# tachitachi/SR-WaveNet

Measured on NVIDIA B200. Metric: audio samples/sec, higher is better.
Workload: dtype f16

## Files before the change

sr-wavenet_b200/csrc/fused_bf16.cu:

```cuda
#include "common.cuh"
#include "mol.cuh"
#include "umma.cuh"
#include "philox.cuh"
#include <cuda_fp16.h>
#include <algorithm>
#include <cstdlib>

const float* srwn_host_weights(srwn_ctx* c);
__global__ void k_cond(const float* __restrict__ enc, const float* __restrict__ cond_k,
                       const float* __restrict__ cond_b, float* __restrict__ cond,
                       int frames_total, int L, int C);

namespace fused {

constexpr int kTile = 128;
#ifndef SRWN_STUDENT_TILES
#define SRWN_STUDENT_TILES 4
#endif
__host__ __device__ constexpr int tiles_of(bool teacher) { return teacher ? 3 : SRWN_STUDENT_TILES; }
__host__ __device__ constexpr int chunk_of(bool teacher) { return kTile * tiles_of(teacher); }
constexpr int kHalo = 512;
constexpr int kMaxLayers = 40;
constexpr int kMaxSeg = 8;

constexpr int kWfBytes = 64 * 32 * 2;
constexpr int kWrsTeacher = 32 * 160 * 2;
constexpr int kWrsStudent = 32 * 32 * 2;
constexpr int kH1Bytes = 128 * 128 * 2;
constexpr int kH2Bytes = 128 * 32 * 2;

struct Seg { int b, t_start, t_out, t_end; };

struct Params {
  const uint8_t* packed;
  const float* x_in;
  const float* x_scored;
  const float* cb;
  uint8_t* rings;
  const Seg* segs;
  const int* nseg;
  uint32_t* flags;
  int G;
  long long wait_limit;
  NoiseSpec noise;
  float* logits_out;
  float* nll_out;
  double* nll_partial;
  float* scale_out;
  float* mean_out;
  float* x_out;
  int* err;
#ifdef SRWN_TUNING
  long long* trace;
  int trace_chunk;
#endif
  int T, L, P, frames, O, M;
  int ring_bytes_per_team;
  int dil[kMaxLayers];
  int ring_off[kMaxLayers];
  int rsuf[kMaxLayers + 1];
};

template <bool TEACHER>
struct SmemMapT {
  static constexpr int NT = tiles_of(TEACHER);
  static constexpr int rows = kHalo + NT * kTile;
  static constexpr int hbuf = 0;
  static constexpr int hbuf_bytes = 4 * rows * 16;
  static constexpr int cbuf = hbuf + 2 * hbuf_bytes;
  static constexpr int cbuf_bytes = 4 * kTile * 16;
  static constexpr int wst = cbuf + NT * cbuf_bytes;
  static constexpr int wst_bytes = kWfBytes + (TEACHER ? kWrsTeacher : kWrsStudent);
  static constexpr int head = wst + 2 * wst_bytes;
  static constexpr int bias = head + (TEACHER ? kH1Bytes + kH2Bytes : 0);
  static constexpr int hbias = bias + kMaxLayers * 32 * 4;
  static constexpr int front = hbias + (128 + 128 + 32 + 64 + 4) * 4;
  static constexpr int cbs = front + 64 * 4;
  static constexpr int bars = cbs + NT * (kMaxLayers + 1) * 32 * 4;
  static constexpr int n_bars = 40;
  static constexpr int misc = bars + n_bars * 8;
  static constexpr int total = misc + 64;
};
static_assert(SmemMapT<true>::total <= 232448 && SmemMapT<false>::total <= 232448, "shared memory budget");
static_assert(3 * 16 * kTile * 16 <= 2 * SmemMapT<true>::hbuf_bytes, "head operand overlay");

template <int NT>
struct BarT {
  static constexpr int D1 = 0;
  static constexpr int D2 = NT;
  static constexpr int HD = 2 * NT;
  static constexpr int WFULL = 4 * NT;
  static constexpr int WEMPTY = WFULL + 2;
  static constexpr int HALO = WFULL + 4;
  static constexpr int G1 = WFULL + 6;
  static constexpr int HDD = WFULL + 8;
  static constexpr int TAIL = HDD + NT;
  static constexpr int C2 = TAIL + 1;
  static constexpr int count = C2 + 2 * NT;
};
static_assert(BarT<3>::count <= 40 && BarT<4>::count <= 40, "barrier slots");

using namespace umma;

template <bool FP16>
__device__ __forceinline__ uint32_t gate2(f2_t a) {
  float a0, a1;
  upk(a, a0, a1);
#if SRWN_EXP & 2
  return pack2<FP16>(a0, a1);
#endif
  const f2_t f = pk(tanh_fast(a0), tanh_fast(a1));
  const f2_t s = mul2(f, f);
  f2_t t = fma2(s, pk(0.0017294071149080992f, 0.0017294071149080992f), pk(-0.020638039335608482f, -0.020638039335608482f));
  t = fma2(s, t, pk(0.2499687224626541f, 0.2499687224626541f));
  const f2_t c = fma2(f, pk(0.5f, 0.5f), mul2(s, t));
  float c0, c1;
  upk(c, c0, c1);
  return pack2<FP16>(c0, c1);
}

template <bool FP16>
__device__ __forceinline__ void store_row(uint8_t* buf, int rows_per_kc, int row, const float* v) {
#pragma unroll
  for (int kc = 0; kc < 4; kc++) {
    uint4 q;
    q.x = pack2<FP16>(v[kc * 8 + 0], v[kc * 8 + 1]); q.y = pack2<FP16>(v[kc * 8 + 2], v[kc * 8 + 3]);
    q.z = pack2<FP16>(v[kc * 8 + 4], v[kc * 8 + 5]); q.w = pack2<FP16>(v[kc * 8 + 6], v[kc * 8 + 7]);
    *reinterpret_cast<uint4*>(buf + ((size_t)kc * rows_per_kc + row) * 16) = q;
  }
}
__device__ __forceinline__ void store_row_packed(uint8_t* buf, int rows_per_kc, int row, const uint32_t* w) {
#pragma unroll
  for (int kc = 0; kc < 4; kc++)
    *reinterpret_cast<uint4*>(buf + ((size_t)kc * rows_per_kc + row) * 16) =
        make_uint4(w[kc * 4 + 0], w[kc * 4 + 1], w[kc * 4 + 2], w[kc * 4 + 3]);
}

#ifndef SRWN_EXP
#define SRWN_EXP 0
#endif
#if !defined(SRWN_TUNING) || !(SRWN_EXP & 16)
#define TRACE(role, layer, slot) do {} while (0)
#else
#define TRACE(role, layer, slot)                                                            \
  do {                                                                                      \
    if (tracing) p.trace[((role) * kMaxLayers + (layer)) * 12 + (slot)] = clock64();      \
  } while (0)
#endif

#if SRWN_EXP & 1
#define LOOP_FENCE() do {} while (0)
#else
#define LOOP_FENCE() fence_async_smem()
#endif

constexpr int kLoadWarp = 0;
__host__ __device__ constexpr int threads_of(bool handoff, int nt) { return (1 + 4 * nt + (handoff ? 1 : 0)) * 32; }

__device__ __noinline__ bool flag_spin(const uint32_t* f, uint32_t need, volatile int* abort_flag, const int* gerr, int code, long long limit) {
  const long long t0 = clock64();
  int spins = 0;
  uint32_t v;
  while (true) {
    __nanosleep(32);
    asm volatile("ld.acquire.gpu.global.u32 %0, [%1];" : "=r"(v) : "l"(f) : "memory");
    if (v >= need) return true;
    if (*abort_flag) return false;
    if (((++spins) & 1023) == 0 && *reinterpret_cast<const volatile int*>(gerr)) return false;
    if (clock64() - t0 > limit) {
      if (atomicCAS((int*)abort_flag, 0, 1) == 0) ((int*)abort_flag)[1] = code;
      return false;
    }
  }
}
__device__ __forceinline__ bool flag_try(const uint32_t* f, uint32_t need) {
  uint32_t v;
  asm volatile("ld.acquire.gpu.global.u32 %0, [%1];" : "=r"(v) : "l"(f) : "memory");
  if (v < need) return false;
  asm volatile("fence.proxy.async;" ::: "memory");
  return true;
}
__device__ __forceinline__ bool flag_wait(const uint32_t* f, uint32_t need, volatile int* abort_flag, const int* gerr, int code, long long limit) {
  uint32_t v;
  asm volatile("ld.acquire.gpu.global.u32 %0, [%1];" : "=r"(v) : "l"(f) : "memory");
  if (v < need && !flag_spin(f, need, abort_flag, gerr, code, limit)) return false;
  asm volatile("fence.proxy.async;" ::: "memory");
  return true;
}
__device__ __forceinline__ void ring_rows_done(uint32_t counter_addr, uint32_t rows) {
  asm volatile("red.release.cta.shared::cta.add.u32 [%0], %1;" ::"r"(counter_addr), "r"(rows) : "memory");
}
__device__ __forceinline__ int ring_rows_of(int d, int m, int chunk) {
  const int lo = max(chunk - d, m * kTile), hi = (m + 1) * kTile;
  return hi > lo ? hi - lo : 0;
}
__device__ __forceinline__ uint32_t ld_acquire_cta_shared(uint32_t addr) {
  uint32_t v;
  asm volatile("ld.acquire.cta.shared::cta.u32 %0, [%1];" : "=r"(v) : "r"(addr) : "memory");
  return v;
}
__device__ __forceinline__ void flag_publish(uint32_t* f, uint32_t chunks) {
  asm volatile("red.release.gpu.global.max.u32 [%0], %1;" ::"l"(f), "r"(chunks) : "memory");
}

template <bool TEACHER, bool FP16, bool HANDOFF>
__global__ void __launch_bounds__(threads_of(HANDOFF, tiles_of(TEACHER)), 1) k_fused(const Params p) {
  constexpr int NT = tiles_of(TEACHER), CH = NT * kTile;
  constexpr int kThreads = threads_of(HANDOFF, NT);
  constexpr int kPubWarp = 1 + 4 * NT;
  constexpr int TCOLS = TEACHER ? 160 : 64;
  using SM = SmemMapT<TEACHER>;
  constexpr int ROWS = SM::rows;
  using BR = BarT<NT>;
  constexpr int BAR_D1 = BR::D1, BAR_D2 = BR::D2, BAR_HD = BR::HD, BAR_WFULL = BR::WFULL, BAR_WEMPTY = BR::WEMPTY, BAR_HALO = BR::HALO,
                BAR_G1 = BR::G1, BAR_HDD = BR::HDD, BAR_TAIL = BR::TAIL, BAR_C2 = BR::C2;
  (void)BAR_HDD; (void)BAR_C2; (void)kPubWarp;
  extern __shared__ __align__(1024) uint8_t smem[];
  const int tid = threadIdx.x, lane = tid & 31, warp = tid >> 5;
  const uint32_t sbase = smem_u32(smem);
  volatile int* abort_flag = reinterpret_cast<volatile int*>(smem + SM::misc + 8);
  uint32_t* tmem_slot = reinterpret_cast<uint32_t*>(smem + SM::misc);
  auto bar = [&](int i) { return sbase + SM::bars + i * 8; };
  const int L = p.L;
  constexpr int wrs_bytes = TEACHER ? kWrsTeacher : kWrsStudent;
  constexpr int layer_bytes = kWfBytes + wrs_bytes;
  constexpr int wrs_rows = TEACHER ? 160 : 32;

  if (tid == 0) {
    for (int i = 0; i < NT; i++) {
      mbar_init(bar(BAR_D1 + i), 1); mbar_init(bar(BAR_D2 + i), 1); mbar_init(bar(BAR_HDD + i), 1);
      mbar_init(bar(BAR_C2 + 2 * i), 1); mbar_init(bar(BAR_C2 + 2 * i + 1), 1);
      mbar_init(bar(BAR_HD + 2 * i), kTile); mbar_init(bar(BAR_HD + 2 * i + 1), kTile);
    }
    for (int i = 0; i < 2; i++) {
      mbar_init(bar(BAR_WFULL + i), 1); mbar_init(bar(BAR_WEMPTY + i), NT);
      mbar_init(bar(BAR_HALO + i), 1); mbar_init(bar(BAR_G1 + i), NT);
    }
    mbar_init(bar(BAR_TAIL), 1);
    abort_flag[0] = 0; abort_flag[1] = 0;
    for (int i = 0; i < NT; i++) reinterpret_cast<volatile uint32_t*>(smem + SM::misc + 16)[i] = 0;
    asm volatile("fence.mbarrier_init.release.cluster;" ::: "memory");
  }
  {
    const uint8_t* pk_ = p.packed;
    const size_t off_fixed = (size_t)L * layer_bytes;
    const float* fbias = reinterpret_cast<const float*>(pk_ + off_fixed);
    float* s_bias = reinterpret_cast<float*>(smem + SM::bias);
    for (int i = tid; i < L * 32; i += kThreads) s_bias[i] = fbias[i];
    const float* ffront = fbias + kMaxLayers * 32;
    float* s_front = reinterpret_cast<float*>(smem + SM::front);
    for (int i = tid; i < 64; i += kThreads) s_front[i] = ffront[i];
    const float* fhb = ffront + 64;
    float* s_hb = reinterpret_cast<float*>(smem + SM::hbias);
    for (int i = tid; i < 128 + 128 + 32 + 64 + 4; i += kThreads) s_hb[i] = fhb[i];
    if (TEACHER) {
      const uint4* src = reinterpret_cast<const uint4*>(reinterpret_cast<const uint8_t*>(fhb + 128 + 128 + 32 + 64 + 4));
      uint4* dst = reinterpret_cast<uint4*>(smem + SM::head);
      for (int i = tid; i < (kH1Bytes + kH2Bytes) / 16; i += kThreads) dst[i] = src[i];
    }
  }
  fence_async_smem();
  if (warp == kLoadWarp) {
    asm volatile("tcgen05.alloc.cta_group::1.sync.aligned.shared::cta.b32 [%0], %1;" ::"r"(smem_u32(tmem_slot)), "r"(512));
    asm volatile("tcgen05.relinquish_alloc_permit.cta_group::1.sync.aligned;" ::);
  }
  tc_fence_before();
  __syncthreads();
  tc_fence_after();
  const uint32_t tmem = *tmem_slot;

  const int G = p.G, team = (int)blockIdx.x / G, member = (int)blockIdx.x % G;
  const Seg* segs = p.segs + (size_t)team * kMaxSeg;
  const int nseg = p.nseg[team];
  uint8_t* ring = p.rings + (size_t)team * p.ring_bytes_per_team;
  uint32_t* flags = p.flags + (size_t)team * kMaxLayers;
  const uint32_t ringcnt = sbase + SM::misc + 16;
  uint32_t pub_expect = 0;
  int seq = 0;
#ifndef SRWN_VAR
#define SRWN_VAR 0
#endif
  constexpr bool handoff = HANDOFF;
  int u0e = 0, u0o = 0, lay_base = 0;
  int chunk_idx = 0;
  int head_idx = 0;
  int tail_idx = 0;
  double nll_acc = 0.0;
  const bool elected = elect_one();

  for (int si = 0; si < nseg; si++) {
    const Seg sg = segs[si];
    for (int t0 = sg.t_start; t0 < sg.t_end; t0 += CH) {
      const int n = seq++;
      if (n % G != member) continue;
      const bool warm = TEACHER ? (t0 + CH <= sg.t_out) : false;
      const bool do_head = TEACHER && !warm;
      int Lc = L;
      if (t0 + CH <= sg.t_out) {
        const int dist = sg.t_out - (t0 + CH);
        Lc = 0;
        while (Lc < L && p.rsuf[Lc + 1] > dist) Lc++;
        if (Lc < 1) Lc = 1;
      }
#define U0(par) ((par) ? u0o : u0e)
#if defined(SRWN_TUNING) && (SRWN_EXP & 16)
      const bool tracing_chunk = p.trace != nullptr && blockIdx.x == 0 && chunk_idx == p.trace_chunk;
#else
      constexpr bool tracing_chunk = false; (void)tracing_chunk;
#endif

      if (warp == kLoadWarp) {
        bool have_next = false;
        for (int l = 0; l < Lc; l++) {
          const int s = l & 1;
          const int use = U0(s) + (l >> 1);
          [[maybe_unused]] const bool tracing = tracing_chunk && lane == 0;
          TRACE(6, l, 0);
          if (l >= 2 && !mbar_wait(bar(BAR_G1 + s), (use - 1) & 1, abort_flag, 0x1100000 | l, p.wait_limit)) break;
          TRACE(6, l, 2);
          if (handoff && !(SRWN_VAR & 2) && n > 0 && !have_next &&
              !flag_wait(flags + l, (uint32_t)n, abort_flag, p.err, 0x1200000 | l, p.wait_limit)) break;
          have_next = false;
          const int d = p.dil[l];
          const uint8_t* rl = ring + p.ring_off[l];
          const uint32_t dst0 = sbase + SM::hbuf + s * SM::hbuf_bytes;
          const int slot0 = (int)((unsigned)t0 % (unsigned)d);
          if (t0 - d >= sg.t_start) {
            if (lane == 0) {
              mbar_expect_tx(bar(BAR_HALO + s), (uint32_t)(4 * d * 16));
              const uint32_t n1 = (uint32_t)(d - slot0) * 16, n2 = (uint32_t)slot0 * 16;
#pragma unroll
              for (int kc = 0; kc < 4; kc++) {
                const uint32_t dst = dst0 + (uint32_t)(kc * ROWS + kHalo - d) * 16;
                const uint8_t* src = rl + (size_t)kc * d * 16;
                asm volatile("cp.async.bulk.shared::cluster.global.mbarrier::complete_tx::bytes [%0], [%1], %2, [%3];"
                             ::"r"(dst), "l"(src + (size_t)slot0 * 16), "r"(n1), "r"(bar(BAR_HALO + s)) : "memory");
                if (n2)
                  asm volatile("cp.async.bulk.shared::cluster.global.mbarrier::complete_tx::bytes [%0], [%1], %2, [%3];"
                               ::"r"(dst + n1), "l"(src), "r"(n2), "r"(bar(BAR_HALO + s)) : "memory");
              }
            }
            __syncwarp();
          } else {
            for (int kc = 0; kc < 4; kc++) {
              for (int i = lane; i < d; i += 32) {
                const uint32_t dst = dst0 + (uint32_t)(kc * ROWS + kHalo - d + i) * 16;
                if (t0 - d + i >= sg.t_start) {
                  int slot = slot0 + i; if (slot >= d) slot -= d;
                  asm volatile("cp.async.cg.shared.global [%0], [%1], 16;" ::"r"(dst), "l"(rl + ((size_t)kc * d + slot) * 16) : "memory");
                } else {
                  asm volatile("st.shared.v4.u32 [%0], {%1, %1, %1, %1};" ::"r"(dst), "r"(0) : "memory");
                }
              }
            }
            asm volatile("cp.async.wait_all;" ::: "memory");
            fence_async_smem();
            __syncwarp();
            if (lane == 0) mbar_arrive(bar(BAR_HALO + s));
          }
          if (handoff && !(SRWN_VAR & 2) && n > 0 && l + 1 < Lc) have_next = flag_try(flags + l + 1, (uint32_t)n);
          if (!mbar_wait(bar(BAR_WEMPTY + s), (use & 1) ^ 1, abort_flag, 0x1000000 | l, p.wait_limit)) break;
          if (lane == 0) {
            mbar_expect_tx(bar(BAR_WFULL + s), layer_bytes);
            asm volatile("cp.async.bulk.shared::cluster.global.mbarrier::complete_tx::bytes [%0], [%1], %2, [%3];"
                         ::"r"(sbase + SM::wst + s * SM::wst_bytes),
                           "l"(p.packed + (size_t)l * layer_bytes), "r"(layer_bytes), "r"(bar(BAR_WFULL + s)) : "memory");
          }
          TRACE(6, l, 1);
          TRACE(6, l, 3);
        }
        if (Lc < L && !*abort_flag) {
          const bool ok = n == 0 || !handoff || (SRWN_VAR & 2) || flag_wait(flags + Lc, (uint32_t)n, abort_flag, p.err, 0x1300000 | Lc, p.wait_limit);
          if (ok && lane == 0) mbar_arrive(bar(BAR_TAIL));
        }
      } else if (HANDOFF && warp == kPubWarp) {
        const int last = Lc < L - 1 ? Lc : L - 1;
        bool ok = handoff && !(SRWN_VAR & 4);
        for (int r = 0; r <= last && ok; r++) {
          if (lane < NT && !(SRWN_VAR & 1)) {
            const int rows = ring_rows_of(p.dil[r], lane, CH);
            if (rows) {
              pub_expect += (uint32_t)rows;
              if ((int32_t)(ld_acquire_cta_shared(ringcnt + 4 * lane) - pub_expect) < 0) {
                const long long t0 = clock64();
                while ((int32_t)(ld_acquire_cta_shared(ringcnt + 4 * lane) - pub_expect) < 0) {
                  __nanosleep((SRWN_VAR & 8) ? 1000 : 128);
                  if (*abort_flag) { ok = false; break; }
                  if (clock64() - t0 > p.wait_limit) {
                    if (atomicCAS((int*)abort_flag, 0, 1) == 0) ((int*)abort_flag)[1] = 0x4000000 | (lane << 8) | r;
                    ok = false; break;
                  }
                }
              }
            }
          }
          ok = __all_sync(0xffffffffu, ok);
          if (ok && lane == 0 && !(SRWN_VAR & 16)) flag_publish(flags + r, (uint32_t)n + 1);
        }
        if (ok && lane == 0)
          for (int r = last + 1; r < L; r++) flag_publish(flags + r, (uint32_t)n + 1);
      } else {
        const int gw = warp & 3, m = (((warp - 1) >> 2) + gw + 1) % NT;
        const bool issuer = gw == m;
        const bool leader = issuer && elected;
        const int row = gw * 32 + lane;
        const uint32_t lane_addr = (uint32_t)(gw * 32) << 16;
        const int t = t0 + m * kTile + row;
        const bool in_utt = t < p.T;
        int frame = (t0 + m * kTile) / p.P;
        if (frame > p.frames - 1) frame = p.frames - 1;
        const float* cb_g = p.cb + ((size_t)sg.b * p.frames + frame) * (size_t)(L + 1) * 32;
        float* cb = reinterpret_cast<float*>(smem + SM::cbs) + m * (kMaxLayers + 1) * 32;
        for (int i = row; i < (L + 1) * 32; i += kTile) cb[i] = __ldg(cb_g + i);
        group_sync(m);
        const float* s_bias = reinterpret_cast<const float*>(smem + SM::bias);
        const float* s_front = reinterpret_cast<const float*>(smem + SM::front);
        const int rc = m * kTile + row;
        f2_t h2[16];
        float v[32];
        uint32_t w16[16];
        bool alive = true;
        [[maybe_unused]] const bool tracing = tracing_chunk && row == 0;
        constexpr uint32_t fmt = FP16 ? 0u : 1u;
        constexpr uint32_t id32 = make_idesc(fmt, 128, 32), id128 = make_idesc(fmt, 128, 128), id160 = make_idesc(fmt, 128, 160); (void)id160;
        const uint32_t hb_lo0 = ((sbase + SM::hbuf) >> 4) + (uint32_t)(kHalo + m * kTile) + ((uint32_t)ROWS << 16);
        const uint32_t wb_lo0 = (sbase + SM::wst) >> 4;
        const uint32_t ab_lo = ((sbase + SM::cbuf + m * SM::cbuf_bytes) >> 4) + ((uint32_t)kTile << 16);
        const uint32_t d_conv = tmem + m * TCOLS, d_skip = tmem + m * TCOLS + 32;
#ifndef SRWN_STUDENT_TMEM_A
#define SRWN_STUDENT_TMEM_A 1
#endif
#ifndef SRWN_STUDENT_LATE_WEMPTY
#define SRWN_STUDENT_LATE_WEMPTY 1
#endif
#ifndef SRWN_LATE_WARP
#define SRWN_LATE_WARP 1
#endif
#ifndef SRWN_STUDENT_LATE_G1
#define SRWN_STUDENT_LATE_G1 1
#endif
#ifndef SRWN_TEACHER_LATE_G1
#define SRWN_TEACHER_LATE_G1 0
#endif
#ifndef SRWN_TEACHER_TMEM_A
#define SRWN_TEACHER_TMEM_A 1
#endif
        constexpr bool kTmemAT = TEACHER && SRWN_TEACHER_TMEM_A;
        constexpr bool kTmemA = (!TEACHER && SRWN_STUDENT_TMEM_A) || kTmemAT;
        uint32_t d_cop = d_skip;
        constexpr bool kLateG1 = TEACHER ? ((SRWN_TEACHER_LATE_G1 == 1 && !HANDOFF) || (SRWN_TEACHER_LATE_G1 == 2 && HANDOFF))
                                         : (!HANDOFF && SRWN_STUDENT_LATE_G1);

        {
          auto x_at = [&](int tt) -> float {
            const size_t i = (size_t)sg.b * p.T + tt;
            if (!TEACHER && p.noise.on) return philox::logistic_at(p.noise.seed, p.noise.stream, (uint64_t)i);
            return __ldg(p.x_in + i);
          };
          const float xm1 = (t >= 1 && t - 1 < p.T) ? x_at(t - 1) : 0.f;
          const float xm2 = (t >= 2 && t - 2 < p.T) ? x_at(t - 2) : 0.f;
#pragma unroll
          for (int j = 0; j < 16; j++) {
            const float a = fmaf(xm2, s_front[2 * j], fmaf(xm1, s_front[32 + 2 * j], cb[2 * j]));
            const float b = fmaf(xm2, s_front[2 * j + 1], fmaf(xm1, s_front[32 + 2 * j + 1], cb[2 * j + 1]));
            h2[j] = pk(a, b);
            w16[j] = pack2<FP16>(a, b);
          }
          alive = mbar_wait(bar(BAR_HALO + 0), U0(0) & 1, abort_flag, 0x2000000 | (m << 8), p.wait_limit);
          store_row_packed(smem + SM::hbuf, ROWS, kHalo + rc, w16);
          const int d0 = p.dil[0];
          fence_async_smem();
          mbar_arrive(bar(BAR_HD + 2 * m + 0));
          if (rc >= CH - d0) store_row_packed(ring + p.ring_off[0], d0, t % d0, w16);
        }

#if defined(SRWN_TUNING) && defined(SRWN_STAGGER)
        if (m > 0) {
          const long long t_go = clock64() + (long long)m * SRWN_STAGGER;
          while (clock64() < t_go) {}
        }
#endif
        for (int l = 0; l < Lc; l++) {
          const int s = l & 1, sn = s ^ 1;
          const uint32_t ph = (lay_base + l) & 1, phs = (U0(s) + (l >> 1)) & 1;
          TRACE(m, l, 0);
          const uint32_t hb_lo = hb_lo0 + (uint32_t)(s * (SM::hbuf_bytes >> 4));
          const uint32_t wb_lo = wb_lo0 + (uint32_t)(s * (SM::wst_bytes >> 4));
          const uint32_t dl = (uint32_t)p.dil[l];
          const uint32_t b1_lo = wb_lo + (32u << 16);
          const uint32_t b2_lo = wb_lo + (kWfBytes >> 4) + ((uint32_t)wrs_rows << 16);
          if (gw == ((m + 3) & 3)) {
            alive = mbar_wait(bar(BAR_WFULL + s), phs, abort_flag, 0x3000000 | (m << 8) | l, p.wait_limit) && alive;
            if (NT > 3 && m >= 3) alive = mbar_wait(bar(BAR_HD + 2 * (m - 3) + s), phs, abort_flag, 0x3300000 | (m << 8) | l, p.wait_limit) && alive;
          }
          if (gw == ((m + 1) & 3) && m >= 1) alive = mbar_wait(bar(BAR_HD + 2 * (m - 1) + s), phs, abort_flag, 0x3100000 | (m << 8) | l, p.wait_limit) && alive;
          if (gw == ((m + 2) & 3) && m >= 2) alive = mbar_wait(bar(BAR_HD + 2 * (m - 2) + s), phs, abort_flag, 0x3200000 | (m << 8) | l, p.wait_limit) && alive;
          group_sync(m);
          TRACE(m, l, 1);
          if (handoff && !(SRWN_VAR & 1) && gw == (m == 0 ? 1 : 0) && lane == 0) {
            const int rows = ring_rows_of((int)dl, m, CH);
            if (rows) ring_rows_done(ringcnt + 4 * m, (uint32_t)rows);
          }
          if (issuer) {
            tc_fence_after();
            if (leader) {
              tc_mma<0>(d_conv, desc_from_lo(hb_lo - dl), desc_from_lo(b1_lo), id32);
              tc_mma<1>(d_conv, desc_from_lo(hb_lo - dl + 2 * ROWS), desc_from_lo(b1_lo + 64), id32);
              tc_mma<1>(d_conv, desc_from_lo(hb_lo), desc_from_lo(b1_lo + 128), id32);
              tc_mma<1>(d_conv, desc_from_lo(hb_lo + 2 * ROWS), desc_from_lo(b1_lo + 192), id32);
              tc_commit(bar(BAR_D1 + m));
              if constexpr (!kLateG1) tc_commit(bar(BAR_G1 + s));
            }
            __syncwarp();
          }
          TRACE(m, l, 2);
          bool next_ok = true;
          if (l + 1 < Lc && !issuer) {
            if (l >= 1) next_ok = mbar_poll(bar(BAR_G1 + sn), (U0(sn) + ((l - 1) >> 1)) & 1);
            next_ok = mbar_poll(bar(BAR_HALO + sn), (U0(sn) + ((l + 1) >> 1)) & 1) && next_ok;
          }

          alive = mbar_wait(bar(BAR_D1 + m), ph, abort_flag, 0x2100000 | (m << 8) | l, p.wait_limit) && alive;
          if (kLateG1 && gw == ((m + 2) & 3) && lane == 0) mbar_arrive(bar(BAR_G1 + s));
          TRACE(m, l, 3);
          tc_fence_after();
          tc_ld32(d_conv + lane_addr, v);
          tc_wait_ld();
          TRACE(m, l, 4);
          {
            const ulonglong2* b2 = reinterpret_cast<const ulonglong2*>(s_bias + l * 32);
            const f2_t neg1 = pk(-1.f, -1.f); (void)neg1;
#pragma unroll
            for (int q = 0; q < 8; q++) {
              const ulonglong2 bb = b2[q];
              const f2_t d0 = pk(v[4 * q], v[4 * q + 1]), d1 = pk(v[4 * q + 2], v[4 * q + 3]);
              w16[2 * q] = gate2<FP16>(add2(d0, bb.x));
              w16[2 * q + 1] = gate2<FP16>(add2(d1, bb.y));
#if SRWN_EXP & 32
              h2[2 * q] = fma2(d0, neg1, h2[2 * q]);
              h2[2 * q + 1] = fma2(d1, neg1, h2[2 * q + 1]);
#endif
            }
          }
          if constexpr (kTmemA) {
            if constexpr (kTmemAT) {
              const int cuse = lay_base + l, prev = m == 2 ? cuse : cuse - 1;
              d_cop = tmem + 480 + 16 * ((cuse + m) & 1);
              if (prev >= 0) alive = mbar_wait(bar(BAR_C2 + 2 * ((m + 1) % 3) + (prev & 1)), (uint32_t)((prev >> 1) & 1), abort_flag, 0x2800000 | (m << 8) | l, p.wait_limit) && alive;
              tc_fence_after();
            }
            tc_st16(d_cop + lane_addr, w16);
            tc_wait_st();
            tc_fence_before();
          } else {
            store_row_packed(smem + SM::cbuf + m * SM::cbuf_bytes, kTile, row, w16);
            tc_fence_before();
            LOOP_FENCE();
          }
          TRACE(m, l, 5);
          next_ok = group_sync_and(m, next_ok);
          TRACE(m, l, 6);
          if (issuer) {
            tc_fence_after();
            if (leader) {
#if SRWN_EXP & 32
              if (TEACHER && !warm && l > 0 && !(SRWN_EXP & 8)) {
                tc_mma<1>(d_conv, desc_from_lo(ab_lo), desc_from_lo(b2_lo), id160);
                tc_mma<1>(d_conv, desc_from_lo(ab_lo + 2 * kTile), desc_from_lo(b2_lo + 2 * wrs_rows), id160);
              } else {
                tc_mma<1>(d_conv, desc_from_lo(ab_lo), desc_from_lo(b2_lo), id32);
                tc_mma<1>(d_conv, desc_from_lo(ab_lo + 2 * kTile), desc_from_lo(b2_lo + 2 * wrs_rows), id32);
                if (TEACHER && !warm && !(SRWN_EXP & 8)) {
                  tc_mma<0>(d_skip, desc_from_lo(ab_lo), desc_from_lo(b2_lo + 32), id128);
                  tc_mma<1>(d_skip, desc_from_lo(ab_lo + 2 * kTile), desc_from_lo(b2_lo + 2 * wrs_rows + 32), id128);
                }
              }
              tc_commit(bar(BAR_D2 + m));
#else
              if constexpr (kTmemA) {
                tc_mma_ts<0>(d_conv, d_cop, desc_from_lo(b2_lo), id32);
                tc_mma_ts<1>(d_conv, d_cop + 8, desc_from_lo(b2_lo + 2 * wrs_rows), id32);
              } else {
                tc_mma<0>(d_conv, desc_from_lo(ab_lo), desc_from_lo(b2_lo), id32);
                tc_mma<1>(d_conv, desc_from_lo(ab_lo + 2 * kTile), desc_from_lo(b2_lo + 2 * wrs_rows), id32);
              }
              tc_commit(bar(BAR_D2 + m));
              if (TEACHER && !warm && !(SRWN_EXP & 8)) {
                if constexpr (kTmemAT) {
                  tc_mma_ts_dyn(d_skip, d_cop, desc_from_lo(b2_lo + 32), id128, l > 0 ? 1u : 0u);
                  tc_mma_ts<1>(d_skip, d_cop + 8, desc_from_lo(b2_lo + 2 * wrs_rows + 32), id128);
                } else {
                  tc_mma_dyn(d_skip, desc_from_lo(ab_lo), desc_from_lo(b2_lo + 32), id128, l > 0 ? 1u : 0u);
                  tc_mma<1>(d_skip, desc_from_lo(ab_lo + 2 * kTile), desc_from_lo(b2_lo + 2 * wrs_rows + 32), id128);
                }
              }
              if constexpr (kTmemAT) tc_commit(bar(BAR_C2 + 2 * m + ((lay_base + l) & 1)));
#endif
#if SRWN_STUDENT_LATE_WEMPTY
              if constexpr (TEACHER || !HANDOFF) tc_commit(bar(BAR_WEMPTY + s));
#else
              tc_commit(bar(BAR_WEMPTY + s));
#endif
            }
            __syncwarp();
          }
          TRACE(m, l, 7);

          alive = mbar_wait(bar(BAR_D2 + m), ph, abort_flag, 0x2200000 | (m << 8) | l, p.wait_limit) && alive;
#if SRWN_STUDENT_LATE_WEMPTY
          if (!TEACHER && HANDOFF && gw == ((m + SRWN_LATE_WARP) & 3) && lane == 0) mbar_arrive(bar(BAR_WEMPTY + s));
#endif
          TRACE(m, l, 8);
          tc_fence_after();
          tc_ld32(d_conv + lane_addr, v);
          tc_wait_ld();
          {
            const ulonglong2* c2 = reinterpret_cast<const ulonglong2*>(cb + (l + 1) * 32);
            const f2_t sq = pk(SRWN_SQRT_HALF, SRWN_SQRT_HALF);
#pragma unroll
            for (int q = 0; q < 8; q++) {
              const ulonglong2 cc = c2[q];
              h2[2 * q] = fma2(add2(h2[2 * q], pk(v[4 * q], v[4 * q + 1])), sq, cc.x);
              h2[2 * q + 1] = fma2(add2(h2[2 * q + 1], pk(v[4 * q + 2], v[4 * q + 3])), sq, cc.y);
            }
          }
          TRACE(m, l, 9);
          if (l + 1 < L) {
#pragma unroll
            for (int j = 0; j < 16; j++) { float a, b; upk(h2[j], a, b); w16[j] = pack2<FP16>(a, b); }
            if (l + 1 < Lc) {
              if (!next_ok) {
                if (l >= 1) alive = mbar_wait(bar(BAR_G1 + sn), (U0(sn) + ((l - 1) >> 1)) & 1, abort_flag, 0x2300000 | (m << 8) | l, p.wait_limit) && alive;
                alive = mbar_wait(bar(BAR_HALO + sn), (U0(sn) + ((l + 1) >> 1)) & 1, abort_flag, 0x2400000 | (m << 8) | l, p.wait_limit) && alive;
              }
              TRACE(m, l, 10);
              store_row_packed(smem + SM::hbuf + sn * SM::hbuf_bytes, ROWS, kHalo + rc, w16);
              tc_fence_before();
              LOOP_FENCE();
              mbar_arrive(bar(BAR_HD + 2 * m + sn));
            } else {
              tc_fence_before();
              alive = mbar_wait(bar(BAR_TAIL), tail_idx & 1, abort_flag, 0x2700000 | (m << 8) | l, p.wait_limit) && alive;
            }
            const int dn = p.dil[l + 1];
            if (rc >= CH - dn) store_row_packed(ring + p.ring_off[l + 1], dn, t % dn, w16);
            TRACE(m, l, 11);
          } else {
            tc_fence_before();
          }
        }

        if (TEACHER) {
          if (do_head) {
            const float* s_hb = reinterpret_cast<const float*>(smem + SM::hbias);
            uint8_t* a3 = smem + SM::hbuf + m * (16 * kTile * 16);
            const uint32_t a3_lo = ((sbase + SM::hbuf + m * (16 * kTile * 16)) >> 4) + ((uint32_t)kTile << 16);
            alive = mbar_wait(bar(BAR_G1 + ((L - 1) & 1)), (U0((L - 1) & 1) + ((L - 1) >> 1)) & 1, abort_flag, 0x2500000 | (m << 8), p.wait_limit) && alive;
            alive = mbar_wait(bar(BAR_WEMPTY + ((L - 1) & 1)), (U0((L - 1) & 1) + ((L - 1) >> 1)) & 1, abort_flag, 0x2510000 | (m << 8), p.wait_limit) && alive;
            tc_fence_after();
#pragma unroll 1
            for (int hs = 0; hs < 2; hs++) {
              for (int q = 0; q < 4; q++) {
                tc_ld32(d_skip + lane_addr + q * 32, v);
                tc_wait_ld();
#pragma unroll
                for (int j = 0; j < 32; j++) v[j] = fmaxf(v[j] + s_hb[hs * 128 + q * 32 + j], 0.f);
                store_row<FP16>(a3 + (size_t)q * 4 * kTile * 16, kTile, row, v);
              }
              tc_fence_before();
              fence_async_smem();
              group_sync(m);
              if (issuer) {
                tc_fence_after();
                if (leader && !*abort_flag) {
                  const uint32_t wlo = ((sbase + SM::head + (hs == 0 ? 0 : kH1Bytes)) >> 4) + ((uint32_t)(hs == 0 ? 128 : 32) << 16);
                  const int nrows = hs == 0 ? 128 : 32;
#pragma unroll
                  for (int j = 0; j < 8; j++)
                    tc_mma_dyn(hs == 0 ? d_skip : d_conv, desc_from_lo(a3_lo + 2 * j * kTile), desc_from_lo(wlo + 2 * j * nrows),
                               hs == 0 ? id128 : id32, j);
                  tc_commit(bar(BAR_HDD + m));
                }
                __syncwarp();
              }
              alive = mbar_wait(bar(BAR_HDD + m), (head_idx * 2 + hs) & 1, abort_flag, 0x2600000 | (m << 8) | hs, p.wait_limit) && alive;
              tc_fence_after();
            }
            tc_ld32(d_conv + lane_addr, v);
            tc_wait_ld();
            tc_fence_before();
            if (alive && in_utt && t >= sg.t_out) {
#pragma unroll
              for (int j = 0; j < 32; j++) v[j] += s_hb[256 + j];
              const size_t at = (size_t)sg.b * p.T + t;
              float nl = 0.f;
              if (p.x_scored) {
                const float xs = __ldg(p.x_scored + at);
                if (p.M == 5) nl = mol_nll_fixed<5>(xs, v);
                else {
                  float lg[32];
#pragma unroll
                  for (int j = 0; j < 32; j++) lg[j] = v[j];
                  nl = mol_nll_one(xs, lg, p.M);
                }
              }
              if (p.logits_out) {
                float* dst = p.logits_out + at * p.O;
                if (p.O == 20) {
#pragma unroll
                  for (int j = 0; j < 5; j++)
                    reinterpret_cast<float4*>(dst)[j] = make_float4(v[4 * j], v[4 * j + 1], v[4 * j + 2], v[4 * j + 3]);
                } else {
#pragma unroll
                  for (int j = 0; j < 32; j++) if (j < p.O) dst[j] = v[j];
                }
              }
              if (p.x_scored) {
                if (p.nll_out) p.nll_out[at] = nl;
                nll_acc += (double)nl;
              }
            }
          }
        } else {
          const float* s_hb = reinterpret_cast<const float*>(smem + SM::hbias);
          const float* hk = s_hb + 288;
          float p0 = 0.f, p1 = 0.f;
#pragma unroll
          for (int j = 0; j < 16; j++) {
            float a, b;
            upk(h2[j], a, b);
            const float e0 = fmaxf(a, 0.f), e1 = fmaxf(b, 0.f);
            p0 = fmaf(e0, hk[4 * j], p0); p1 = fmaf(e0, hk[4 * j + 1], p1);
            p0 = fmaf(e1, hk[4 * j + 2], p0); p1 = fmaf(e1, hk[4 * j + 3], p1);
          }
          if (alive && in_utt && t >= sg.t_out) {
            const size_t at = (size_t)sg.b * p.T + t;
            const float sc = expf(p0 + hk[64]);
            const float mu = p1 + hk[65];
            p.scale_out[at] = sc;
            p.mean_out[at] = mu;
            const float xin = p.noise.on ? philox::logistic_at(p.noise.seed, p.noise.stream, (uint64_t)at) : __ldg(p.x_in + at);
            p.x_out[at] = fmaf(xin, sc, mu);
          }
        }
      }
      if (handoff && !(SRWN_VAR & 1) && Lc < L && warp != kLoadWarp && warp != kPubWarp) {
        const int gw = warp & 3, m = (((warp - 1) >> 2) + gw + 1) % NT;
        group_sync(m);
        if (gw == (m == 0 ? 1 : 0) && lane == 0) {
          const int rows = ring_rows_of(p.dil[Lc], m, CH);
          if (rows) ring_rows_done(ringcnt + 4 * m, (uint32_t)rows);
        }
      }
      if (do_head) head_idx++;
      if (Lc < L) tail_idx++;
      chunk_idx++;
      u0e += (Lc + 1) >> 1; u0o += Lc >> 1; lay_base += Lc;
      tc_fence_before();
      asm volatile("fence.proxy.async;" ::: "memory");
      __syncthreads();
      tc_fence_after();
      if (*abort_flag) break;
    }
    if (*abort_flag) break;
  }

  if (TEACHER && p.nll_partial) {
    double* s_red = reinterpret_cast<double*>(smem + SM::cbuf);
    for (int s = 16; s >= 1; s >>= 1) nll_acc += __shfl_xor_sync(0xffffffffu, nll_acc, s);
    if (lane == 0) s_red[warp] = nll_acc;
    __syncthreads();
    if (tid == 0) {
      double tot = 0;
      for (int w = 1; w <= 4 * NT; w++) tot += s_red[w];
      p.nll_partial[blockIdx.x] = tot;
    }
  }
  if (tid == 0 && *abort_flag) {
    volatile int* e = p.err;
    e[1] = abort_flag[1]; e[2] = chunk_idx; e[3] = blockIdx.x;
    __threadfence_system();
    e[0] = 1;
  }
  tc_fence_before();
  __syncthreads();
  if (warp == kLoadWarp) {
    tc_fence_after();
    asm volatile("tcgen05.dealloc.cta_group::1.sync.aligned.b32 %0, %1;" ::"r"(tmem), "r"(512));
  }
}

__global__ void k_sum_partials(const double* __restrict__ part, int n, float* __restrict__ out) {
  double tot = 0;
  for (int i = threadIdx.x; i < n; i += 32) tot += part[i];
  for (int s = 16; s >= 1; s >>= 1) tot += __shfl_xor_sync(0xffffffffu, tot, s);
  if (threadIdx.x == 0) *out = (float)tot;
}

__global__ void k_fold_bias(const float* __restrict__ cond, const float* __restrict__ front_b,
                            const float* __restrict__ res_b, float* __restrict__ cb, int L) {
  const int bf = blockIdx.x;
  for (int o = threadIdx.x; o < (L + 1) * 32; o += blockDim.x) {
    const int i = o / 32, j = o % 32;
    float v = i < L ? cond[((size_t)bf * L + i) * 32 + j] : 0.f;
    v += i == 0 ? front_b[j] : SRWN_SQRT_HALF * res_b[(i - 1) * 32 + j];
    cb[(size_t)bf * (L + 1) * 32 + o] = v;
  }
}


#ifndef SRWN_COND_ROWS
#define SRWN_COND_ROWS 16
#endif
constexpr int kCondRows = SRWN_COND_ROWS;
constexpr int kCondRowsPerThread = 16;
constexpr int kCondThreads = 256 * (kCondRows / kCondRowsPerThread);
static_assert(kCondRows % kCondRowsPerThread == 0 && kCondRows >= kCondRowsPerThread, "SRWN_COND_ROWS is a multiple of 16");
__global__ void __launch_bounds__(kCondThreads, 512 / kCondThreads)
k_cond_fold(const float* __restrict__ enc, const float* __restrict__ cond_k, const float* __restrict__ cond_b,
            const float* __restrict__ front_b, const float* __restrict__ res_b, float* __restrict__ cb,
            int BF, int L, int C, size_t w_stride, size_t cb_stride) {
  constexpr int RH = kCondRowsPerThread;
  {
    const size_t wo = (size_t)blockIdx.y * w_stride;
    cond_k += wo; cond_b += wo; front_b += wo; res_b += wo; cb += (size_t)blockIdx.y * cb_stride;
  }
  __shared__ __align__(16) float s_enc[kCondRows][kMaxCond];
  const int bf0 = blockIdx.x * kCondRows;
  for (int i = threadIdx.x; i < kCondRows * kMaxCond; i += blockDim.x) {
    const int r = i / kMaxCond, c = i % kMaxCond;
    s_enc[r][c] = (bf0 + r < BF && c < C) ? enc[(size_t)(bf0 + r) * C + c] : 0.f;
  }
  __syncthreads();
  const int half = threadIdx.x / 256, r0 = half * RH;
  for (int g = threadIdx.x % 256; g < (L + 1) * 8; g += 256) {
    const int l = g / 8, j = (g % 8) * 4, o = l * 32 + j;
    float4 base;
    {
      const float4 cbv = l < L ? *reinterpret_cast<const float4*>(cond_b + l * 32 + j) : make_float4(0.f, 0.f, 0.f, 0.f);
      if (l == 0) {
        const float4 f = *reinterpret_cast<const float4*>(front_b + j);
        base = make_float4(cbv.x + f.x, cbv.y + f.y, cbv.z + f.z, cbv.w + f.w);
      } else {
        const float4 rb = *reinterpret_cast<const float4*>(res_b + (l - 1) * 32 + j);
        base = make_float4(cbv.x + SRWN_SQRT_HALF * rb.x, cbv.y + SRWN_SQRT_HALF * rb.y, cbv.z + SRWN_SQRT_HALF * rb.z, cbv.w + SRWN_SQRT_HALF * rb.w);
      }
    }
    float4 acc[RH];
#pragma unroll
// ... 226 lines not shown
    r.xa = w.take<float>(n);
    r.xb = w.take<float>(n);
  }
  r.bytes = w.used;
  return r;
}

size_t fused_partition_bytes(const srwn_ctx* c) {
  const size_t grid = c->sm_count > 0 ? c->sm_count : 148;
  return grid * kMaxSeg * sizeof(Seg) + grid * sizeof(int);
}

size_t fused_workspace_bytes(const srwn_ctx* c, int op, int B, int T) {
  return carve_fused(c, B, T, nullptr, 0).bytes;
}

template <bool TEACHER>
static int launch_fused(srwn_ctx* c, const Params& p, int grid, int fp16, cudaStream_t st) {
  if (!fp16) return srwn_fail(SRWN_ERR_UNSUPPORTED, "the fused kernel is built for fp16 operands only (bf16 misses the 2e-2 logit bound)");
  const bool handoff = p.G > 1;
  auto kern = handoff ? k_fused<TEACHER, true, true> : k_fused<TEACHER, true, false>;
  SRWN_CUDA(cudaFuncSetAttribute(kern, cudaFuncAttributeMaxDynamicSharedMemorySize, SmemMapT<TEACHER>::total));
  Params pl = p;
  void* args[] = {&pl};
  SRWN_CUDA(cudaLaunchCooperativeKernel((const void*)kern, dim3(grid), dim3(threads_of(handoff, tiles_of(TEACHER))), args, SmemMapT<TEACHER>::total, st));
  SRWN_LAUNCH_CHECK();
  return SRWN_OK;
}

static int sticky_error(const srwn_ctx* c) {
  const volatile int* e = c->h_err;
  if (e && e[0])
    return srwn_fail(SRWN_ERR_CUDA, "an earlier fused launch aborted: pipeline wait timed out (code 0x%x, chunk %d, cta %d); "
                     "results of that call are invalid", e[1], e[2], e[3]);
  return SRWN_OK;
}

static int prepare(srwn_ctx* c, int stack, const float* enc, int B, int T, const FusedWs& w, Params* p,
                   int* grid, bool first, int fp16, cudaStream_t st) {
  const int L = c->cfg.n_layers, P = c->cfg.pool_stride, frames = T / P;
  const float* sw = stack_w(c, stack);
  int rc = sticky_error(c);
  if (rc) return rc;
  const int nst = c->cfg.kind == SRWN_STUDENT ? c->cfg.num_flows : 1;
  const size_t cb_stride = (size_t)B * frames * (L + 1) * 32, flag_stride = (size_t)c->sm_count * kMaxLayers;
  if (first) {
    const float* s0 = stack_w(c, 0);
    k_cond_fold<<<dim3((B * frames + kCondRows - 1) / kCondRows, nst), kCondThreads, 0, st>>>(
        enc, s0 + c->off.cond_k, s0 + c->off.cond_b, s0 + c->off.front_b, s0 + c->off.res_b, w.cb, B * frames, L,
        c->cfg.cond_channels, c->stack_floats, cb_stride);
    SRWN_LAUNCH_CHECK();
    SRWN_CUDA(cudaMemsetAsync(w.flags, 0, flag_stride * nst * sizeof(uint32_t), st));
  }
  (void)sw;
  const size_t seg_bytes = (size_t)c->sm_count * kMaxSeg * sizeof(Seg), n_bytes = (size_t)c->sm_count * sizeof(int);
  if (first && (c->part_B != B || c->part_T != T || c->part_team_req != c->team_size)) {
    const bool teacher = c->cfg.kind == SRWN_TEACHER;
    Partition part = make_partition(B, T, chunk_of(teacher), teacher ? 1.10 : 1.04, c->dilations, c->sm_count, c->team_size);
    c->part_host.assign(seg_bytes + n_bytes, 0);
    memcpy(c->part_host.data(), part.segs.data(), std::min(seg_bytes, part.segs.size() * sizeof(Seg)));
    memcpy(c->part_host.data() + seg_bytes, part.nseg.data(), std::min(n_bytes, part.nseg.size() * sizeof(int)));
    SRWN_CUDA(cudaMemcpyAsync(c->d_part, c->part_host.data(), c->part_host.size(), cudaMemcpyHostToDevice, st));
    c->part_B = B; c->part_T = T; c->part_team_req = c->team_size;
    c->part_teams = part.teams; c->part_G = part.G;
  }
  *grid = c->part_teams * c->part_G;
  memset(p, 0, sizeof(*p));
  const size_t img = stack_image_bytes(c);
  p->packed = (const uint8_t*)c->d_packed + ((size_t)(fp16 ? 1 : 0) * c->n_stacks + stack) * img;
  p->cb = w.cb + (size_t)stack * cb_stride; p->rings = w.rings; p->flags = w.flags + (size_t)stack * flag_stride; p->err = c->h_err; p->G = c->part_G;
  p->wait_limit = c->wait_limit_clocks;
  p->segs = reinterpret_cast<const Seg*>(c->d_part);
  p->nseg = reinterpret_cast<const int*>(reinterpret_cast<const uint8_t*>(c->d_part) + seg_bytes);
  p->T = T; p->L = L; p->P = P; p->frames = frames;
  p->O = 4 * c->cfg.num_mixtures; p->M = c->cfg.num_mixtures;
  p->ring_bytes_per_team = c->sum_dilation * 64 + 256;
  int off = 0;
  for (int l = 0; l < L; l++) { p->dil[l] = c->dilations[l]; p->ring_off[l] = off; off += c->dilations[l] * 64; }
  p->rsuf[L] = 0;
  for (int l = L - 1; l >= 0; l--) p->rsuf[l] = p->rsuf[l + 1] + c->dilations[l];
#ifdef SRWN_TUNING
  p->trace = getenv("SRWN_TRACE") ? w.trace : nullptr;
  p->trace_chunk = getenv("SRWN_TRACE") ? atoi(getenv("SRWN_TRACE")) : 0;
#endif
  return SRWN_OK;
}

int run_teacher_fused_bf16(srwn_ctx* c, const float* x_in, const float* enc, const float* x_scored,
                           float* nll_out, float* nll_sum, float* logits_out, int B, int T, int fp16,
                           void* ws, size_t ws_bytes, cudaStream_t st) {
  if (!fused_supported(c)) return srwn_fail(SRWN_ERR_UNSUPPORTED, "fused 16-bit path needs dilations <= %d, layers <= %d, pool_stride %% 128 == 0", kHalo, kMaxLayers);
  FusedWs w = carve_fused(c, B, T, ws, ws_bytes);
  if (!ws || w.bytes > ws_bytes) return srwn_fail(SRWN_ERR_WORKSPACE, "workspace too small: need %zu bytes", w.bytes);
  Params p;
  int grid = 0;
  int rc = prepare(c, 0, enc, B, T, w, &p, &grid, true, fp16, st);
  if (rc) return rc;
  p.x_in = x_in; p.x_scored = x_scored; p.logits_out = logits_out; p.nll_out = nll_out;
  p.nll_partial = (x_scored && nll_sum) ? w.partial : nullptr;
  {
    ProfScope prof(c, st, "k_fused<teacher,fp16>", 1);
    rc = launch_fused<true>(c, p, grid, fp16, st);
    if (rc) return rc;
  }
  if (p.nll_partial) {
    k_sum_partials<<<1, 32, 0, st>>>(w.partial, grid, nll_sum);
    SRWN_LAUNCH_CHECK();
  }
  return SRWN_OK;
}

int run_student_fused_bf16(srwn_ctx* c, const float* z, NoiseSpec noise, float* z_out, const float* enc, float* out, float* s_tot,
                           float* mu_tot, float* x_last, int B, int T, int fp16, void* ws, size_t ws_bytes,
                           cudaStream_t st) {
  if (!fused_supported(c)) return srwn_fail(SRWN_ERR_UNSUPPORTED, "fused 16-bit path needs dilations <= %d, layers <= %d, pool_stride %% 128 == 0", kHalo, kMaxLayers);
  FusedWs w = carve_fused(c, B, T, ws, ws_bytes);
  if (!ws || w.bytes > ws_bytes) return srwn_fail(SRWN_ERR_WORKSPACE, "workspace too small: need %zu bytes", w.bytes);
  const size_t n = (size_t)B * T;
  const int F = c->cfg.num_flows;
  const float* xin = z;
  int grid = 0;
  for (int f = 0; f < F; f++) {
    Params p;
    int rc = prepare(c, f, enc, B, T, w, &p, &grid, f == 0, fp16, st);
    if (rc) return rc;
    float* xout = (f == F - 1 && x_last) ? x_last : ((f & 1) ? w.xb : w.xa);
    p.x_in = xin; p.scale_out = w.scales + (size_t)f * n; p.mean_out = w.means + (size_t)f * n; p.x_out = xout;
    if (f == 0) p.noise = noise;
    ProfScope prof(c, st, "k_fused<student,fp16>", 1);
    rc = launch_fused<false>(c, p, grid, fp16, st);
    if (rc) return rc;
    xin = xout;
  }
  return run_flow_compose(z, noise, z_out, w.scales, w.means, F, out, s_tot, mu_tot, (int64_t)n, st);
}

int fused_check_error(void* ws, size_t ws_bytes, const srwn_ctx* c, int B, int T, cudaStream_t st) {
  (void)ws; (void)ws_bytes; (void)B; (void)T;
  SRWN_CUDA(cudaStreamSynchronize(st));
  volatile int* e = c->h_err;
  if (e && e[0]) {
    const int code = e[1], chunk = e[2], cta = e[3];
    e[0] = 0; e[1] = 0; e[2] = 0; e[3] = 0;
    return srwn_fail(SRWN_ERR_CUDA, "fused kernel aborted: pipeline wait timed out (code 0x%x, chunk %d, cta %d)", code, chunk, cta);
  }
  return SRWN_OK;
}

void fused_last_partition(const srwn_ctx* c, int* teams, int* G) { *teams = c->part_teams; *G = c->part_G; }

#ifdef SRWN_TUNING
extern "C" int srwn_debug_read_trace(srwn_handle_t h, int32_t B, int32_t T, void* ws, size_t ws_bytes,
                                     long long* out, int32_t count) {
  FusedWs w = carve_fused(h, B, T, ws, ws_bytes);
  if (count > 7 * kMaxLayers * 12) count = 7 * kMaxLayers * 12;
  SRWN_CUDA(cudaDeviceSynchronize());
  SRWN_CUDA(cudaMemcpy(out, w.trace, sizeof(long long) * count, cudaMemcpyDeviceToHost));
  return SRWN_OK;
}

namespace fused {
template <int N, int CNT>
__device__ __forceinline__ void bench_issue(uint32_t tmem_col, uint32_t a_lo, uint32_t b_lo, uint32_t mbar_addr) {
  constexpr uint32_t idesc = make_idesc(0, 128, N);
#pragma unroll
  for (int i = 0; i < CNT; i++) {
// ... 83 lines not shown
```

Before: 909.3 million.

## Prefetch next chunk's conditioning bias and input samples via cp.async in teacher path

For the teacher path without handoff, each compute group now issues cp.async loads for the next chunk's conditioning-bias row and its tile of input samples (with a two-sample causal lead) while the output head's MMA is running, or right after a group sync when there is no head. The current chunk then only waits on those loads instead of doing synchronous __ldg reads, and it reads x[t-1] and x[t-2] from shared memory. The goal is to hide global-load latency at each chunk start. It adds tracing hooks and assumes the shared cbuf region is free during the prefetch window, which is a risk if anything else still uses it.

Result: faster. 919.7 million (median of 6 runs) (+1.1%).

```diff
diff --git a/sr-wavenet_b200/csrc/fused_bf16.cu b/sr-wavenet_b200/csrc/fused_bf16.cu
--- a/sr-wavenet_b200/csrc/fused_bf16.cu
+++ b/sr-wavenet_b200/csrc/fused_bf16.cu
@@ -52,7 +52,7 @@
   int* err;
 #ifdef SRWN_TUNING
   long long* trace;
-  int trace_chunk;
+  int trace_chunk, trace_cta;
 #endif
   int T, L, P, frames, O, M;
   int ring_bytes_per_team;
@@ -141,11 +141,17 @@
 #endif
 #if !defined(SRWN_TUNING) || !(SRWN_EXP & 16)
 #define TRACE(role, layer, slot) do {} while (0)
+#define TRACE_AT(on, role, layer, slot) do {} while (0)
 #else
 #define TRACE(role, layer, slot)                                                            \
   do {                                                                                      \
     if (tracing) p.trace[((role) * kMaxLayers + (layer)) * 12 + (slot)] = clock64();      \
   } while (0)
+#define TRACE_AT(on, role, layer, slot)                                                     \
+  do {                                                                                      \
+    if (on) p.trace[((role) * kMaxLayers + (layer)) * 12 + (slot)] = clock64();            \
+  } while (0)
+constexpr int kPhaseRow = kMaxLayers - 1, kNextRow = kMaxLayers - 2;
 #endif
 
 #if SRWN_EXP & 1
@@ -287,6 +293,19 @@
   int tail_idx = 0;
   double nll_acc = 0.0;
   const bool elected = elect_one();
+  auto next_chunk = [&](int si, int t0, int n, int& b, int& tn) -> bool {
+    Seg s = segs[si];
+    for (;;) {
+      t0 += CH; n++;
+      while (t0 >= s.t_end) {
+        if (++si >= nseg) return false;
+        s = segs[si]; t0 = s.t_start;
+      }
+      if (n % G == member) { b = s.b; tn = t0; return true; }
+    }
+  };
+  constexpr bool kPrefetch = TEACHER && !HANDOFF;
+  bool loads_issued = false;
 
   for (int si = 0; si < nseg; si++) {
     const Seg sg = segs[si];
@@ -304,9 +323,10 @@
       }
 #define U0(par) ((par) ? u0o : u0e)
 #if defined(SRWN_TUNING) && (SRWN_EXP & 16)
-      const bool tracing_chunk = p.trace != nullptr && blockIdx.x == 0 && chunk_idx == p.trace_chunk;
+      const bool tracing_chunk = p.trace != nullptr && (int)blockIdx.x == p.trace_cta && chunk_idx == p.trace_chunk;
+      const bool tracing_next = p.trace != nullptr && (int)blockIdx.x == p.trace_cta && chunk_idx == p.trace_chunk + 1;
 #else
-      constexpr bool tracing_chunk = false; (void)tracing_chunk;
+      constexpr bool tracing_chunk = false, tracing_next = false; (void)tracing_chunk; (void)tracing_next;
 #endif
 
       if (warp == kLoadWarp) {
@@ -315,6 +335,7 @@
           const int s = l & 1;
           const int use = U0(s) + (l >> 1);
           [[maybe_unused]] const bool tracing = tracing_chunk && lane == 0;
+          if (l == 0) TRACE_AT(tracing_next && lane == 0, 6, kNextRow, 0);
           TRACE(6, l, 0);
           if (l >= 2 && !mbar_wait(bar(BAR_G1 + s), (use - 1) & 1, abort_flag, 0x1100000 | l, p.wait_limit)) break;
           TRACE(6, l, 2);
@@ -340,6 +361,7 @@
                                ::"r"(dst + n1), "l"(src), "r"(n2), "r"(bar(BAR_HALO + s)) : "memory");
               }
             }
+            if (l == 0) TRACE_AT(tracing_next && lane == 0, 6, kNextRow, 1);
             __syncwarp();
           } else {
             for (int kc = 0; kc < 4; kc++) {
@@ -366,9 +388,11 @@
                          ::"r"(sbase + SM::wst + s * SM::wst_bytes),
                            "l"(p.packed + (size_t)l * layer_bytes), "r"(layer_bytes), "r"(bar(BAR_WFULL + s)) : "memory");
           }
+          if (l == 0) TRACE_AT(tracing_next && lane == 0, 6, kNextRow, 2);
           TRACE(6, l, 1);
           TRACE(6, l, 3);
         }
+        TRACE_AT(tracing_chunk && lane == 0, 6, kPhaseRow, 0);
         if (Lc < L && !*abort_flag) {
           const bool ok = n == 0 || !handoff || (SRWN_VAR & 2) || flag_wait(flags + Lc, (uint32_t)n, abort_flag, p.err, 0x1300000 | Lc, p.wait_limit);
           if (ok && lane == 0) mbar_arrive(bar(BAR_TAIL));
@@ -411,8 +435,37 @@
         if (frame > p.frames - 1) frame = p.frames - 1;
         const float* cb_g = p.cb + ((size_t)sg.b * p.frames + frame) * (size_t)(L + 1) * 32;
         float* cb = reinterpret_cast<float*>(smem + SM::cbs) + m * (kMaxLayers + 1) * 32;
-        for (int i = row; i < (L + 1) * 32; i += kTile) cb[i] = __ldg(cb_g + i);
+        const uint32_t sx_u32 = sbase + SM::cbuf + m * SM::cbuf_bytes;
+        auto issue_loads = [&](int b, int tc0) {
+          int fr = (tc0 + m * kTile) / p.P;
+          if (fr > p.frames - 1) fr = p.frames - 1;
+          const float* src = p.cb + ((size_t)b * p.frames + fr) * (size_t)(L + 1) * 32;
+          for (int i = row; i < (L + 1) * 8; i += kTile)
+            asm volatile("cp.async.cg.shared.global [%0], [%1], 16;" ::"r"(sbase + SM::cbs + (uint32_t)(m * (kMaxLayers + 1) * 32 + 4 * i) * 4),
+                         "l"(src + 4 * i) : "memory");
+          for (int j = row; j < kTile + 2; j += kTile) {
+            const int tt = tc0 + m * kTile - 2 + j;
+            if (tt >= 0 && tt < p.T)
+              asm volatile("cp.async.ca.shared.global [%0], [%1], 4;" ::"r"(sx_u32 + 4 * j), "l"(p.x_in + (size_t)b * p.T + tt) : "memory");
+            else
+              asm volatile("st.shared.f32 [%0], %1;" ::"r"(sx_u32 + 4 * j), "f"(0.f) : "memory");
+          }
+        };
+        auto prefetch_next = [&]() {
+          int nb, nt0;
+          if (next_chunk(si, t0, n, nb, nt0)) { issue_loads(nb, nt0); loads_issued = true; }
+        };
+        (void)cb_g; (void)issue_loads; (void)prefetch_next;
+        TRACE_AT(tracing_next && row == 0, m, kNextRow, 0);
+        if constexpr (kPrefetch) {
+          if (!loads_issued) issue_loads(sg.b, t0);
+          loads_issued = false;
+          asm volatile("cp.async.wait_all;" ::: "memory");
+        } else {
+          for (int i = row; i < (L + 1) * 32; i += kTile) cb[i] = __ldg(cb_g + i);
+        }
         group_sync(m);
+        TRACE_AT(tracing_next && row == 0, m, kNextRow, 1);
         const float* s_bias = reinterpret_cast<const float*>(smem + SM::bias);
         const float* s_front = reinterpret_cast<const float*>(smem + SM::front);
         const int rc = m * kTile + row;
@@ -457,8 +510,14 @@
             if (!TEACHER && p.noise.on) return philox::logistic_at(p.noise.seed, p.noise.stream, (uint64_t)i);
             return __ldg(p.x_in + i);
           };
-          const float xm1 = (t >= 1 && t - 1 < p.T) ? x_at(t - 1) : 0.f;
-          const float xm2 = (t >= 2 && t - 2 < p.T) ? x_at(t - 2) : 0.f;
+          float xm1, xm2;
+          if constexpr (kPrefetch) {
+            const float* sx = reinterpret_cast<const float*>(smem + SM::cbuf + m * SM::cbuf_bytes);
+            xm1 = sx[row + 1]; xm2 = sx[row];
+          } else {
+            xm1 = (t >= 1 && t - 1 < p.T) ? x_at(t - 1) : 0.f;
+            xm2 = (t >= 2 && t - 2 < p.T) ? x_at(t - 2) : 0.f;
+          }
 #pragma unroll
           for (int j = 0; j < 16; j++) {
             const float a = fmaf(xm2, s_front[2 * j], fmaf(xm1, s_front[32 + 2 * j], cb[2 * j]));
@@ -466,7 +525,9 @@
             h2[j] = pk(a, b);
             w16[j] = pack2<FP16>(a, b);
           }
+          TRACE_AT(tracing_next && row == 0, m, kNextRow, 2);
           alive = mbar_wait(bar(BAR_HALO + 0), U0(0) & 1, abort_flag, 0x2000000 | (m << 8), p.wait_limit);
+          TRACE_AT(tracing_next && row == 0, m, kNextRow, 3);
           store_row_packed(smem + SM::hbuf, ROWS, kHalo + rc, w16);
           const int d0 = p.dil[0];
           fence_async_smem();
@@ -496,6 +557,7 @@
           if (gw == ((m + 1) & 3) && m >= 1) alive = mbar_wait(bar(BAR_HD + 2 * (m - 1) + s), phs, abort_flag, 0x3100000 | (m << 8) | l, p.wait_limit) && alive;
           if (gw == ((m + 2) & 3) && m >= 2) alive = mbar_wait(bar(BAR_HD + 2 * (m - 2) + s), phs, abort_flag, 0x3200000 | (m << 8) | l, p.wait_limit) && alive;
           group_sync(m);
+          if (l == 0) TRACE_AT(tracing_next && row == 0, m, kNextRow, 4);
           TRACE(m, l, 1);
           if (handoff && !(SRWN_VAR & 1) && gw == (m == 0 ? 1 : 0) && lane == 0) {
             const int rows = ring_rows_of((int)dl, m, CH);
@@ -513,6 +575,7 @@
             }
             __syncwarp();
           }
+          if (l == 0) TRACE_AT(tracing_next && issuer && elected, m, kNextRow, 5);
           TRACE(m, l, 2);
           bool next_ok = true;
           if (l + 1 < Lc && !issuer) {
@@ -650,6 +713,7 @@
           }
         }
 
+        TRACE_AT(tracing, m, kPhaseRow, 0);
         if (TEACHER) {
           if (do_head) {
             const float* s_hb = reinterpret_cast<const float*>(smem + SM::hbias);
@@ -657,6 +721,7 @@
             const uint32_t a3_lo = ((sbase + SM::hbuf + m * (16 * kTile * 16)) >> 4) + ((uint32_t)kTile << 16);
             alive = mbar_wait(bar(BAR_G1 + ((L - 1) & 1)), (U0((L - 1) & 1) + ((L - 1) >> 1)) & 1, abort_flag, 0x2500000 | (m << 8), p.wait_limit) && alive;
             alive = mbar_wait(bar(BAR_WEMPTY + ((L - 1) & 1)), (U0((L - 1) & 1) + ((L - 1) >> 1)) & 1, abort_flag, 0x2510000 | (m << 8), p.wait_limit) && alive;
+            TRACE_AT(tracing, m, kPhaseRow, 1);
             tc_fence_after();
 #pragma unroll 1
             for (int hs = 0; hs < 2; hs++) {
@@ -670,6 +735,7 @@
               tc_fence_before();
               fence_async_smem();
               group_sync(m);
+              TRACE_AT(tracing, m, kPhaseRow, 2 + 2 * hs);
               if (issuer) {
                 tc_fence_after();
                 if (leader && !*abort_flag) {
@@ -683,12 +749,15 @@
                 }
                 __syncwarp();
               }
+              if (kPrefetch && hs == 0) prefetch_next();
               alive = mbar_wait(bar(BAR_HDD + m), (head_idx * 2 + hs) & 1, abort_flag, 0x2600000 | (m << 8) | hs, p.wait_limit) && alive;
+              TRACE_AT(tracing, m, kPhaseRow, 3 + 2 * hs);
               tc_fence_after();
             }
             tc_ld32(d_conv + lane_addr, v);
             tc_wait_ld();
             tc_fence_before();
+            TRACE_AT(tracing, m, kPhaseRow, 6);
             if (alive && in_utt && t >= sg.t_out) {
 #pragma unroll
               for (int j = 0; j < 32; j++) v[j] += s_hb[256 + j];
@@ -720,6 +789,10 @@
                 nll_acc += (double)nl;
               }
             }
+            TRACE_AT(tracing, m, kPhaseRow, 7);
+          } else if (kPrefetch) {
+            group_sync(m);
+            prefetch_next();
           }
         } else {
           const float* s_hb = reinterpret_cast<const float*>(smem + SM::hbias);
@@ -758,13 +831,18 @@
       u0e += (Lc + 1) >> 1; u0o += Lc >> 1; lay_base += Lc;
       tc_fence_before();
       asm volatile("fence.proxy.async;" ::: "memory");
+      [[maybe_unused]] const bool trace_bar = tracing_chunk && lane == 0 && (warp == kLoadWarp || ((warp & 3) == 0 && warp <= 4 * NT));
+      [[maybe_unused]] const int trace_role = warp == kLoadWarp ? 6 : (((warp - 1) >> 2) + 1) % NT;
+      TRACE_AT(trace_bar, trace_role, kPhaseRow, 8);
       __syncthreads();
+      TRACE_AT(trace_bar, trace_role, kPhaseRow, 9);
       tc_fence_after();
       if (*abort_flag) break;
     }
     if (*abort_flag) break;
   }
 
+  if constexpr (kPrefetch) asm volatile("cp.async.wait_all;" ::: "memory");
   if (TEACHER && p.nll_partial) {
     double* s_red = reinterpret_cast<double*>(smem + SM::cbuf);
     for (int s = 16; s >= 1; s >>= 1) nll_acc += __shfl_xor_sync(0xffffffffu, nll_acc, s);
@@ -1157,6 +1235,7 @@
 #ifdef SRWN_TUNING
   p->trace = getenv("SRWN_TRACE") ? w.trace : nullptr;
   p->trace_chunk = getenv("SRWN_TRACE") ? atoi(getenv("SRWN_TRACE")) : 0;
+  p->trace_cta = getenv("SRWN_TRACE_CTA") ? atoi(getenv("SRWN_TRACE_CTA")) : 0;
 #endif
   return SRWN_OK;
 }
```
